# ryought/dbgphmm

Measured on AMD Instinct MI355X. Metric: read-bases/sec through forward+backward P(R|X), higher is better.
Workload: dtype f64

## Files before the change

dbgphmm_amd/_ffi.py:

```python
from __future__ import annotations

import ctypes as C
import os
import subprocess

_HERE = os.path.dirname(os.path.abspath(__file__))
LIB_PATH = os.environ.get("PHMM_AMD_LIB") or os.path.join(_HERE, "libphmm_amd.so")
CSRC = os.path.join(_HERE, "csrc")

PHMM_OK, PHMM_EINVAL, PHMM_ENODEVICE, PHMM_ENOMEM, PHMM_ECAPACITY, PHMM_EINTERNAL = 0, -1, -2, -3, -4, -5
PHMM_GROUP_MIXED = 0xFFFFFFFF
PHMM_STATS_DENSE_FWD, PHMM_STATS_DENSE_BWD, PHMM_STATS_SPARSE_FWD, PHMM_STATS_SPARSE_BWD, PHMM_STATS_HINTED_WIDE = range(5)
PHMM_READ_DEFERRED, PHMM_READ_WIDE_FRONTIER, PHMM_READ_FORCED_SWITCH = 1, 2, 4


class PhmmError(RuntimeError):
    def __init__(self, code: int, msg: str):
        super().__init__(f"phmm_amd error {code}: {msg}")
        self.code = code


def build(force: bool = False) -> str:
    if force:
        subprocess.check_call(["make", "-C", CSRC, "-s", "clean"])
# ... 59 lines not shown
        "phmm_full_prob_reads_copy_num_changes": (i32, [vp, vp, vp, vp, u32, u32, vp, vp, vp, vp, vp, vp]),
        "phmm_likelihood_create": (i32, [vp, vp, vp, vp, u32, P(vp)]),
        "phmm_likelihood_score_changes": (i32, [vp, u32, vp, vp, vp, vp, vp, vp]),
        "phmm_likelihood_move": (i32, [vp, u64, vp, vp, vp, vp]),
        "phmm_likelihood_current": (i32, [vp, vp, vp, vp]),
        "phmm_likelihood_refresh": (i32, [vp]),
        "phmm_likelihood_destroy": (None, [vp]),
        "phmm_likelihood_set_groups": (i32, [vp, u32, vp, vp]),
        "phmm_likelihood_score_group_changes": (i32, [vp, u32, vp, vp, vp, vp, vp, vp]),
        "phmm_likelihood_move_groups": (i32, [vp, u64, vp, vp, vp, vp]),
        "phmm_likelihood_current_groups": (i32, [vp, vp]),
        "phmm_generate_mappings": (i32, [vp, vp, vp, i32, P(vp), vp]),
        "phmm_run_with_mapping_edges": (i32, [vp, vp, vp, vp, vp, vp]),
        "phmm_last_call_stats": (i32, [i32, P(dbl), P(u64), P(u64)]),
        "phmm_enable_timing": (i32, [i32]),
    }
    for name, (res, args) in sig.items():
        fn = getattr(L, name)
        fn.restype = res
        fn.argtypes = args
    _lib = L
    return L


DECLARED_SYMBOLS = [
    "phmm_last_error", "phmm_version", "phmm_device_count", "phmm_set_device", "phmm_set_stream",
    "phmm_set_workspace_limit", "phmm_release_workspace", "phmm_workspace_bytes", "phmm_reads_last_call_info", "phmm_params_new", "phmm_params_uniform", "phmm_model_create",
    "phmm_model_set_probs", "phmm_model_set_params", "phmm_model_n_nodes", "phmm_model_n_edges",
    "phmm_model_destroy", "phmm_reads_create", "phmm_reads_count", "phmm_reads_total_bases",
    "phmm_reads_destroy", "phmm_run_dense", "phmm_run_dense_edges", "phmm_q_score_exact", "phmm_run_sparse", "phmm_full_prob_sparse_backward", "phmm_backward_sparse_tables", "phmm_dense_tables", "phmm_mappings_create",
# ... 6 lines not shown
    "phmm_likelihood_refresh", "phmm_likelihood_destroy",
    "phmm_likelihood_set_groups", "phmm_likelihood_score_group_changes", "phmm_likelihood_move_groups",
    "phmm_likelihood_current_groups",
]


def check(rc: int) -> None:
    if rc != PHMM_OK:
        raise PhmmError(rc, lib().phmm_last_error().decode())


def last_call_stats(which: int):
    ms, n, c = C.c_double(), C.c_uint64(), C.c_uint64()
    check(lib().phmm_last_call_stats(which, C.byref(ms), C.byref(n), C.byref(c)))
    return ms.value, n.value, c.value
```

dbgphmm_amd/csrc/api.cpp:

```cpp
#include <chrono>
#include <cstdlib>
#include <cmath>
#include <cstring>

#include "phmm_internal.h"

namespace phmm {

static thread_local std::string g_error;
static thread_local hipStream_t g_stream = nullptr;
static thread_local uint64_t g_ws_limit = 0;
static thread_local CallStats g_stats;
static thread_local bool g_timing = false;

void set_error(const std::string &msg) { g_error = msg; }
int fail(int code, const std::string &msg) {
    g_error = msg;
    return code;
}
hipStream_t current_stream() { return g_stream; }
int &workset_index() {
    static thread_local int idx = 0;
    return idx;
}
// ... 42 lines not shown
    k.no_wide_hinted = flag("PHMM_NO_WIDE_HINTED");
    k.wide_hinted = flag("PHMM_WIDE_HINTED") && !k.no_wide_hinted;
    k.no_wide_list_bwd = flag("PHMM_NO_WIDE_LIST_BWD");
    k.wide_hinted_cpb = num("PHMM_WIDE_HINTED_CPB", 0);
    if (k.wide_hinted_cpb != 1 && k.wide_hinted_cpb != 2 && k.wide_hinted_cpb != 4) k.wide_hinted_cpb = 0;
    k.no_side_worker = flag("PHMM_NO_SIDE_WORKER");
    k.no_wide_handover = flag("PHMM_NO_WIDE_HANDOVER");
    k.workers = std::max(1, std::min(MAX_WORKERS, num("PHMM_WORKERS", 1)));
    k.warm_cols = num("PHMM_WARM_COLS", 0);
    k.chunk_groups = std::max(0, num("PHMM_CHUNK_GROUPS", 0));
    k.no_keep_all = flag("PHMM_NO_KEEP_ALL");
    k.pipeline_min_groups = std::max(1, num("PHMM_PIPELINE_MIN_GROUPS", 8));
    k.no_runmax = flag("PHMM_NO_RUNMAX");
    k.force_radix = flag("PHMM_FORCE_RADIX");
    k.no_bwd_skip = flag("PHMM_NO_BWD_SKIP");
    k.serial_emit = flag("PHMM_SERIAL_EMIT");
    k.emit_high_priority = flag("PHMM_EMIT_HIGH_PRIORITY");
    k.no_dma = flag("PHMM_NO_DMA");
    k.bwd_dma = flag("PHMM_BWD_DMA");
    k.dense_streams = num("PHMM_DENSE_STREAMS", 0);
    k.dense_w = num("PHMM_DENSE_W", 0);
    k.dense_npt = num("PHMM_DENSE_NPT", 0);
    if (const char *e = std::getenv("PHMM_MEM_FRACTION")) k.mem_fraction = std::min(0.97, std::max(0.1, std::atof(e)));
    g_knobs = k;
}

void trace(const char *tag) {
    if (!g_knobs.trace) return;
    static thread_local std::chrono::steady_clock::time_point last = std::chrono::steady_clock::now();
    (void)hipStreamSynchronize(g_stream);
// ... 216 lines not shown
}
int phmm_set_workspace_limit(uint64_t bytes) {
    g_ws_limit = bytes;
    return PHMM_OK;
}
int phmm_enable_timing(int on) {
    g_timing = on != 0;
    return PHMM_OK;
}
int phmm_last_call_stats(int which, double *ms, uint64_t *launches, uint64_t *cells) {
    if (which < 0 || which > 4) return fail(PHMM_EINVAL, "which out of range");
    if (ms) *ms = g_stats.ms[which];
    if (launches) *launches = g_stats.launches[which];
    if (cells) *cells = g_stats.cells[which];
    return PHMM_OK;
}

static double lnz(double x) { return x > 0.0 ? std::log(x) : -INFINITY; }

int phmm_params_new(double p_mismatch, double p_gap_open, double p_gap_ext, double p_end,
                    int64_t n_active_nodes, int64_t n_warmup, phmm_params *o) {
    return guarded([&] {
        if (!o) PHMM_THROW(PHMM_EINVAL, "out is NULL");
        o->p_mismatch = lnz(p_mismatch);
        o->p_gap_open = lnz(p_gap_open);
        o->p_gap_ext = lnz(p_gap_ext);
        o->p_end = lnz(p_end);
        o->p_DD = o->p_II = o->p_gap_ext;
        o->p_MI = o->p_MD = o->p_ID = o->p_DI = o->p_gap_open;
        const double go = std::exp(o->p_gap_open), ge = std::exp(o->p_gap_ext), pe = std::exp(o->p_end);
// ... 650 lines not shown
```

dbgphmm_amd/csrc/dense.hip:

```cpp
#include <algorithm>
#include <cmath>
#include <cstring>
#include <numeric>
#include <type_traits>

#include "dense_internal.h"
#include "lds_dma.h"

#ifndef PHMM_FWD_PF
#define PHMM_FWD_PF 2
#endif
#ifndef PHMM_BWD_PF
#define PHMM_BWD_PF 1
#endif
#ifndef PHMM_SMALLW_WAVES
#define PHMM_SMALLW_WAVES 3
#endif

namespace phmm {


__device__ __forceinline__ int xcd_block(int b, int nblk8) {
    int per = nblk8 >> 3;
    return (b & 7) * per + (b >> 3);
// ... 749 lines not shown
    const double t2 = block_reduce_rows<W>(s2, OpAdd(), lds);
    if (threadIdx.x < W && lb < a.nblk) {
        double *bp = a.bpart + ((size_t)(pos & 1) * a.ng + g) * a.nblk8 * W * 2;
        bp[((size_t)lb * W + r) * 2 + 0] = t1;
        bp[((size_t)lb * W + r) * 2 + 1] = t2;
    }
    if (lb == 0 && threadIdx.x < W && live) a.BE[((size_t)g * (a.Lc + 1) + pos) * W + r] = Epos;
}

template <int W>
__global__ void __launch_bounds__(BLOCK) bwd_finish(const DenseArgs a) {
    __shared__ double lds[(BLOCK / 64) * 64];
    bwd_chain<W>(a, blockIdx.x, 0, lds);
}

__global__ void __launch_bounds__(BLOCK) freq_reduce(const double *accg, int ng, int N, double *out, int accumulate) {
    const int k = blockIdx.x * BLOCK + threadIdx.x;
    if (k >= N) return;
    double s = accumulate ? out[k] : 0.0;
    for (int g = 0; g < ng; g++) s += accg[(size_t)g * N + k];
    out[k] = s;
}

template <int W>
__global__ void __launch_bounds__(BLOCK) edge_freq_kernel(const DenseArgs a, const uint32_t *esrc, const uint32_t *edst,
                                                          const double *trans, const double *init, int E, double *accE,
                                                          double *accI) {
    constexpr int ROWS = BLOCK / W;
    const int g = blockIdx.y;
    const int r = threadIdx.x % W, row = threadIdx.x / W;
// ... 294 lines not shown
        if (w == 1 || w == 2 || w == 4 || w == 8 || w == 16 || w == 32 || w == 64) p.W = w;
    }
    p.ng_total = (int)((R + p.W - 1) / p.W);
    const int rows = BLOCK / p.W;
    int npt = 8;
    const double lanes_total = (double)m->N * (double)(p.ng_total * p.W);
    while (npt < 64 && lanes_total / (npt * 2) >= 524288.0) npt *= 2;
    while ((int64_t)((m->N + (int64_t)npt * rows - 1) / ((int64_t)npt * rows)) > 4096 && npt < 64) npt *= 2;
    if (knobs().dense_npt > 0) npt = std::max(2, std::min(256, knobs().dense_npt & ~1));
    p.npt = npt;
    p.nblk = (int)((m->N + (int64_t)npt * rows - 1) / ((int64_t)npt * rows));
    p.nblk8 = (p.nblk + 7) / 8 * 8;
    return p;
}

void layout(DenseArgs &a, int W, bool full_b, void *tables, void *misc, size_t &tb, size_t &mb, bool backward_only) {
    const size_t NW = (size_t)a.N * W;
    Carver t(tables), s(misc);
    const size_t fcols = backward_only ? 0 : (size_t)a.Lc;
    a.Fm = t.take<double>((size_t)a.ng * fcols * NW);
    a.Fi = t.take<double>((size_t)a.ng * fcols * NW);
    a.Fd = t.take<double>((size_t)a.ng * fcols * NW);
    a.bcols = full_b ? a.Lc : 2;
    a.Bm = t.take<double>((size_t)a.ng * a.bcols * NW);
    a.Bi = t.take<double>((size_t)a.ng * a.bcols * NW);
    a.Bd = (full_b || backward_only) ? t.take<double>((size_t)a.ng * a.bcols * NW) : nullptr;
    tb = t.off;
    a.bases = s.take<uint8_t>((size_t)a.ng * a.Lc * W);
    a.len = s.take<int>((size_t)a.ng * W);
    a.FE = s.take<int>((size_t)a.ng * (a.Lc + 1) * W);
    a.BE = s.take<int>((size_t)a.ng * (a.Lc + 1) * W);
    a.cmaxF = s.take<unsigned long long>((size_t)a.ng * a.Lc * W);
    a.cmaxB = s.take<unsigned long long>((size_t)a.ng * a.Lc * W);
    a.epart = s.take<double>((size_t)a.ng * (a.eall ? a.Lc : 1) * a.nblk8 * W);
    a.logPf = s.take<double>((size_t)a.ng * W);
    a.logE = s.take<double>(a.eall ? (size_t)a.ng * a.Lc * W : 1);
    a.bpart = s.take<double>((size_t)2 * a.ng * a.nblk8 * W * 2);
    a.logmbB = s.take<double>((size_t)a.ng * (a.Lc + 1) * W);
    a.logibB = s.take<double>((size_t)a.ng * (a.Lc + 1) * W);
    a.accg = s.take<double>((size_t)a.ng * a.N);
    a.logib = s.take<double>((size_t)a.Lc + 1);
    a.tmaxF = s.take<unsigned long long>((size_t)a.ng * a.Lc * W);
// ... 383 lines not shown
```

dbgphmm_amd/csrc/dense_internal.h:

```cpp
#pragma once

#include <vector>

#include "phmm_internal.h"
#include "seg_hull.h"

namespace phmm {

static constexpr double LN2 = 0.693147180559945309417232121458;
static constexpr int BLOCK = 256;

struct DenseArgs {
    int N, ng, Lc, nblk, npt;
    int g_off;
    const NodeRec *nodes;
    const uint8_t *emis;
    const double *init, *dinit, *tdinit;
    const uint32_t *fc_off;
    const FwdEntry *fc;
    const uint32_t *bc_off;
    const BwdEntry *bc;
    const uint32_t *fh_off, *bh_off;
    const HopEntry *fh, *bh;
    int hop_mode;
// ... 36 lines not shown
    uint8_t *skA = nullptr;
    int nrun = 0, nseg = 0, sseg = 1;
    unsigned long long *skcells = nullptr;
};
static constexpr int WF_CAP = 1024;


struct Plan {
    int W, ng_total, npt, nblk, nblk8;
    std::vector<uint32_t> order;
};

Plan make_plan(const phmm_model *m, const phmm_reads *reads, int forced_w);
Plan make_plan_ids(const phmm_model *m, const phmm_reads *reads, const std::vector<uint32_t> &ids);
void layout(DenseArgs &a, int W, bool full_b, void *tables, void *misc, size_t &tb, size_t &mb,
            bool backward_only = false);
void fill_model_args(DenseArgs &a, const phmm_model *m);
void host_logib(const phmm_model *m, size_t n, std::vector<double> &out);
void launch_fwd_step(int W, const DenseArgs &a, int pos);
void launch_fwd_finish(int W, const DenseArgs &a);
void launch_bwd_step(int W, const DenseArgs &a, int pos);
void launch_bwd_finish(int W, const DenseArgs &a);

struct ExactTables {
    double *f_m, *f_i, *f_d, *f_scal, *b_m, *b_i, *b_d, *b_scal;
};
void exact_dense_reads(phmm_model *m, const uint8_t *bases, const uint64_t *off, const std::vector<uint32_t> &ids, double *lf,
                       double *lb, double *freq_dev, const ExactTables *tabs, double *edge_freq_dev = nullptr,
                       double *init_freq_dev = nullptr);
bool certify_dense(int N, int len, double log2P, const int *FE, const double *log2maxF, const int *BE, const double *log2maxB,
                   double log2_p_end);
// ... 4 lines not shown
```

dbgphmm_amd/csrc/mapping_flow.hip:

```cpp
#include <algorithm>
#include <cmath>
#include <cstring>
#include <memory>

#include <hipcub/hipcub.hpp>

#include "sparse_dyn.h"
#include "lean_bwd_kernel.h"
#include "wide_bwd_kernel.h"

namespace phmm {

static constexpr int KMAX = PHMM_MAX_ACTIVE_NODES;

template <int CAP> struct FRec {
    double m[CAP], i[CAP], d[CAP];
    uint32_t id[CAP];
    int n, na, E;
};

template <int CAP> __device__ bool load_record(const RecPool &p, uint64_t pos_index, FRec<CAP> &f) {
    const uint64_t o1 = p.off[pos_index];
    if (o1 == 0) return false;
    const uint8_t *rec = p.base + (o1 - 8);
// ... 884 lines not shown
        pos_max = std::max(pos_max, hb[gi] & ~(1 << 30));
    }
    DevBuf &ctl = m->wset().aux[3], &pbuf = m->wset().aux[4];
    const bool skip = W == 64 && !knobs().no_bwd_skip && pos_max >= 0;
    const int sseg = seg_size(mc.a.npt);
    const RunSucc *rsucc = skip ? &model_run_successors(m, sseg) : nullptr;
    const size_t sk_nrun = ((size_t)m->N + mc.a.npt - 1) / mc.a.npt;
    size_t cb = 0;
    auto carve = [&](size_t bytes) {
        cb = (cb + 255) / 256 * 256;
        size_t o = cb;
        cb += bytes;
        return o;
    };
    const size_t o_bs = carve(sizeof(int) * lanes), o_ca = carve(sizeof(int) * lanes * 2), o_cb = carve(sizeof(int) * lanes * 2),
                 o_err = carve(sizeof(uint32_t) * lanes), o_cells = carve(sizeof(unsigned long long)), o_lanes = carve(sizeof(uint32_t) * std::max<size_t>(sparse_lanes.size(), 1)),
                 o_lp0 = carve(sizeof(uint64_t) * (lanes + 1)), o_gp0 = carve(sizeof(uint64_t) * (lanes + 1)),
                 o_stop = carve(sizeof(int) * lanes),
                 o_skh = carve(skip ? sizeof(uint32_t) * (size_t)mc.a.ng * rsucc->nseg : 0), o_ska = carve(skip ? 2 * (size_t)mc.a.ng * sk_nrun : 0),
                 o_bn = carve(sizeof(uint32_t) * (size_t)lanes * KMAX * 2), o_bv = carve(sizeof(double) * (size_t)lanes * KMAX * 2),
                 o_an = carve(sizeof(uint32_t) * (size_t)lanes * KMAX * 2), o_av = carve(sizeof(double) * (size_t)lanes * KMAX * 2),
                 o_hand = carve(sizeof(BHandoff) * (size_t)lanes), o_eoff = carve(sizeof(unsigned long long) * 2 * (size_t)lanes),
                 o_wls = carve(sizeof(uint32_t) * 2 * (size_t)lanes), o_wlb = carve(sizeof(uint32_t) * 2 * (size_t)lanes),
                 o_wlc = carve(sizeof(int) * 2), o_lb = carve(sizeof(double) * (size_t)lanes);
    ctl.reserve(cb);
    char *cp = (char *)ctl.p;
    const size_t prun_n = (size_t)mc.ngc * mc.a.nblk8 * BLOCK;
    bool need_pb = false;
    for (int gi = 0; gi < lanes; gi++) need_pb |= hb[gi] >= 0 && !(hb[gi] & (1 << 30));
    pbuf.reserve(((need_pb ? 3 : 2) * (size_t)mc.ngc * NW + prun_n) * sizeof(double));
    unsigned long long top_before = 0;
    HIP_CHECK(hipMemcpyAsync(&top_before, sink->mp.top, sizeof(top_before), hipMemcpyDeviceToHost, s));
    HIP_CHECK(hipStreamSynchronize(s));

    for (int attempt = 0;; attempt++) {
        HIP_CHECK(hipMemsetAsync(cp, 0, o_bn, s));
        HIP_CHECK(hipMemcpyAsync(cp + o_bs, hb.data(), sizeof(int) * lanes, hipMemcpyHostToDevice, s));
        HIP_CHECK(hipMemcpyAsync(cp + o_lp0, lp0.data(), sizeof(uint64_t) * (lanes + 1), hipMemcpyHostToDevice, s));
        HIP_CHECK(hipMemcpyAsync(cp + o_gp0, gp0.data(), sizeof(uint64_t) * (lanes + 1), hipMemcpyHostToDevice, s));
        if (!sparse_lanes.empty())
            HIP_CHECK(hipMemcpyAsync(cp + o_lanes, sparse_lanes.data(), sizeof(uint32_t) * sparse_lanes.size(),
                                     hipMemcpyHostToDevice, s));
        const RecPool mp = sink->mp;

        DenseArgs a = mc.a;
        a.want_freq = 0;
        a.want_map = 1;
        a.bstart = (const int *)(cp + o_bs);
        a.Pa = pbuf.as<double>();
        a.Pb = need_pb ? pbuf.as<double>() + 2 * (size_t)mc.ngc * NW : pbuf.as<double>();
        a.Prun = knobs().no_runmax ? nullptr : pbuf.as<double>() + (need_pb ? 3 : 2) * (size_t)mc.ngc * NW;
        const bool st_on = W == 64 && mc.main_plan;
        if (skip) {
            a.rs_off = rsucc->off.as<uint32_t>();
            a.rs = rsucc->ent.as<uint32_t>();
            a.nseg = (int)rsucc->nseg;
            a.sseg = sseg;
            a.nrun = (int)sk_nrun;
            a.skH = (uint32_t *)(cp + o_skh);
            a.skA = (uint8_t *)(cp + o_ska);
            a.skcells = st_on ? (unsigned long long *)(cp + o_cells) : nullptr;
            HIP_CHECK(hipMemsetAsync(pbuf.p, 0, sizeof(double) * 2 * (size_t)mc.ngc * NW, s));
        }
        HIP_CHECK(hipMemsetAsync(a.cmaxB, 0, sizeof(unsigned long long) * (size_t)a.ng * a.Lc * W, s));
        HIP_CHECK(hipMemsetAsync(a.pmax, 0, sizeof(unsigned long long) * (size_t)a.ng * (a.Lc + 1) * W, s));
        HIP_CHECK(hipMemsetAsync(a.BE, 0, sizeof(int) * (size_t)a.ng * (a.Lc + 1) * W, s));
        HIP_CHECK(hipMemsetAsync(a.Bm, 0, sizeof(double) * (size_t)a.ng * a.bcols * NW, s));
        HIP_CHECK(hipMemsetAsync(a.Bi, 0, sizeof(double) * (size_t)a.ng * a.bcols * NW, s));

        if (!sparse_lanes.empty()) {
            hipLaunchKernelGGL(merge_logp, dim3((unsigned)((sparse_lanes.size() + BLOCK - 1) / BLOCK)), dim3(BLOCK), 0, s,
                               (const uint32_t *)(cp + o_lanes), (int)sparse_lanes.size(), mc.d_logp_sparse, a.logPf);
            SparseBwdArgs ba{};
            ba.M = mc.fa_M;
            ba.d = a;
            ba.W = W;
            ba.Lb = mc.Lfull;
            ba.sw = mc.d_sw;
            ba.bases = mc.d_bases_full;
            ba.fpool = mc.fpool;
            ba.mpool = mp;
            ba.lane_pos0 = (const uint64_t *)(cp + o_lp0);
            ba.map_pos0 = (const uint64_t *)(cp + o_gp0);
// ... 91 lines not shown
        std::unique_lock<std::mutex> dense_lock;
        if (mc.dense_token) dense_lock = std::unique_lock<std::mutex>(*mc.dense_token);
        const int wi = workset_index();
        if (!m->pool->cstream[wi]) {
            int least = 0, greatest = 0;
            HIP_CHECK(hipDeviceGetStreamPriorityRange(&least, &greatest));
            HIP_CHECK(hipStreamCreateWithPriority(&m->pool->cstream[wi], hipStreamNonBlocking, knobs().emit_high_priority ? greatest : least));
        }
        for (auto &e : m->pool->cevent[wi])
            if (!e) HIP_CHECK(hipEventCreateWithFlags(&e, hipEventDisableTiming));
        hipStream_t s2 = knobs().serial_emit ? s : m->pool->cstream[wi];
        hipEvent_t *ev_col = &m->pool->cevent[wi][0], *ev_emit = &m->pool->cevent[wi][2];
        bool emitted[2] = {false, false};
        for (int pos = pos_max; pos >= 0; pos--) {
            const int par = pos & 1;
            a.Pa = pbuf.as<double>() + (size_t)par * mc.ngc * NW;
            ma.d = a;
            ma.cntA = (int *)(cp + o_ca) + (size_t)par * lanes;
            ma.cntB = (int *)(cp + o_cb) + (size_t)par * lanes;
            ma.candA_node = (uint32_t *)(cp + o_an) + (size_t)par * lanes * KMAX;
            ma.candA_val = (double *)(cp + o_av) + (size_t)par * lanes * KMAX;
            ma.candB_node = (uint32_t *)(cp + o_bn) + (size_t)par * lanes * KMAX;
            ma.candB_val = (double *)(cp + o_bv) + (size_t)par * lanes * KMAX;
            if (emitted[par]) HIP_CHECK(hipStreamWaitEvent(s, ev_emit[par], 0));
            lt.begin();
            launch_bwd_step(W, a, pos);
            lt.end();
            launch_post_collect_w(W, ma, pos);
            HIP_CHECK(hipEventRecord(ev_col[par], s));
            HIP_CHECK(hipStreamWaitEvent(s2, ev_col[par], 0));
            hipLaunchKernelGGL(emit_offsets, dim3(1), dim3(1024), 0, s2, ma, pos, lanes);
            {
                const int ub = std::max(1, live_at[(size_t)pos] * (need_pb ? 2 : 1));
                hipLaunchKernelGGL(emit_dense_small, dim3((unsigned)std::min(1024, (ub + BLOCK / 64 - 1) / (BLOCK / 64))), dim3(BLOCK), 0,
                                   s2, ma, pos, lanes);
                hipLaunchKernelGGL(emit_dense_map, dim3((unsigned)ub), dim3(BLOCK), 0, s2, ma, pos, lanes);
            }
            HIP_CHECK(hipEventRecord(ev_emit[par], s2));
            emitted[par] = true;
            if (st_on) st.launches[1]++;
        }
        for (int par = 0; par < 2; par++)
            if (emitted[par]) HIP_CHECK(hipStreamWaitEvent(s, ev_emit[par], 0));
        HIP_CHECK(hipGetLastError());
        const bool want_lb = mc.logb_out && pos_max >= 0 && lanes > 0;
        if (want_lb) {
            launch_bwd_finish(W, a);
            hipLaunchKernelGGL(gather_logb, dim3((unsigned)((lanes + BLOCK - 1) / BLOCK)), dim3(BLOCK), 0, s, (const double *)a.logmbB,
                               a.Lc, W, lanes, (double *)(cp + o_lb));
            HIP_CHECK(hipGetLastError());
        }
        st.ms[1] += lt.total_ms();
        for (int gi = 0; gi < lanes; gi++)
            if (st_on && !a.skcells && hb[gi] >= 0) st.cells[1] += (uint64_t)((hb[gi] & ~(1 << 30)) + 1) * m->N;
        const size_t err_words = (o_cells + sizeof(unsigned long long) - o_err) / sizeof(uint32_t);
        std::vector<uint32_t> herr(err_words);
        HIP_CHECK(hipMemcpyAsync(herr.data(), cp + o_err, sizeof(uint32_t) * err_words, hipMemcpyDeviceToHost, s));
        if (want_lb) HIP_CHECK(hipMemcpyAsync(mc.logb_out, cp + o_lb, sizeof(double) * lanes, hipMemcpyDeviceToHost, s));
        HIP_CHECK(hipStreamSynchronize(s));
        if (a.skcells) {
            unsigned long long nc = 0;
            memcpy(&nc, herr.data() + (o_cells - o_err) / sizeof(uint32_t), sizeof nc);
            st.cells[1] += nc;
        }
        if (dense_lock.owns_lock()) dense_lock.unlock();
        trace("  dense backward+collect");
        bool pool_full = false;
        for (int gi = 0; gi < lanes; gi++) {
            if (herr[gi] & SP_ERR_POOL) pool_full = true;
            else if (herr[gi] & ~SP_STOP_SLICE) PHMM_THROW(PHMM_EINTERNAL, "mapping backward error " + std::to_string(herr[gi]));
        }
        if (!pool_full) break;
        (void)attempt;
        throw SinkOverflow{};
    }
}

__global__ void __launch_bounds__(BLOCK) map_counts(RecPool mp, uint64_t n_pos, uint64_t *cnt) {
    const uint64_t p = (uint64_t)blockIdx.x * BLOCK + threadIdx.x;
    if (p > n_pos) return;
    uint64_t c = 0;
    if (p < n_pos) {
        const uint64_t o1 = mp.off[p];
        if (o1) c = ((const uint32_t *)(mp.base + (o1 - 8)))[0];
    }
    cnt[p] = c;
}
__global__ void __launch_bounds__(BLOCK) map_compact(RecPool mp, uint64_t n_pos, const uint64_t *pos_off, uint32_t *nodes,
                                                     double *logp) {
    const uint64_t p = (uint64_t)blockIdx.x * BLOCK + threadIdx.x;
// ... 692 lines not shown
```

dbgphmm_amd/csrc/phmm_internal.h:

```cpp
#pragma once

#include <hip/hip_runtime.h>

#include <cstdint>
#include <cstdio>
#include <memory>
#include <mutex>
#include <string>
#include <vector>

#include "../../include/phmm_amd.h"

namespace phmm {

void set_error(const std::string &msg);
int fail(int code, const std::string &msg);

struct Error {
    int code;
    std::string msg;
};
#define PHMM_THROW(code, msg) throw ::phmm::Error{(code), (msg)}
#define HIP_CHECK(expr)                                                                      \
    do {                                                                                     \
// ... 48 lines not shown
    }
    void *detach() {
        void *q = p;
        p = nullptr;
        bytes = 0;
        return q;
    }
    template <class T> T *as() const { return reinterpret_cast<T *>(p); }
    void upload(const void *src, size_t n) {
        reserve(n);
        if (n) HIP_CHECK(hipMemcpyAsync(p, src, n, hipMemcpyHostToDevice, current_stream()));
    }
};
void copy_out(void *dst, const void *src_dev, size_t bytes);

struct WorkSet {
    DevBuf tables, misc, aux[24];
    size_t bytes() const {
        size_t b = tables.bytes + misc.bytes;
        for (const auto &a : aux) b += a.bytes;
        return b;
    }
    void release() {
        tables.release();
        misc.release();
        for (auto &a : aux) a.release();
    }
};
static constexpr int MAX_WORKERS = 4;
struct DevicePool {
    int device = 0;
    std::recursive_mutex call_mu;
    WorkSet wsets[MAX_WORKERS];
    hipStream_t wstream[MAX_WORKERS] = {};
    hipStream_t cstream[MAX_WORKERS] = {};
    hipEvent_t cevent[MAX_WORKERS][4] = {};
    DevBuf ws_out;
    static constexpr size_t SPARE_MAX = 6, SPARE_BYTES = (size_t)8 << 30;
    std::mutex spare_mu;
    std::vector<std::pair<void *, size_t>> spare;
// ... 2 lines not shown
    void take(DevBuf &b, size_t n);
    void flush_spares();
    size_t owned_table_bytes() const {
        size_t b = 0;
        for (const auto &w : wsets) b += w.tables.bytes;
        return b;
    }
    size_t owned_bytes() const {
        size_t b = ws_out.bytes + spare_total;
        for (const auto &w : wsets) b += w.bytes();
        return b;
    }
    void release();
};
DevicePool &device_pool();

struct LinParams {
    double p_mismatch, p_match, p_random, p_end;
    double p_MM, p_IM, p_DM, p_MI, p_II, p_DI, p_MD, p_ID, p_DD;
    int n_max_gaps;
};

struct FwdEntry {
    uint32_t node;
    uint32_t pad;
    double w1, wD, wT;
};
struct BwdEntry {
    uint32_t node;
    uint32_t emis;
// ... 133 lines not shown
    std::vector<uint32_t> g_of;
    std::vector<uint32_t> g_cn;
    std::vector<uint32_t> g_emit;
    std::vector<uint32_t> g_seen;
    std::vector<uint32_t> g_at;
    uint32_t g_stamp = 0;
    phmm::DevBuf d_g_off, d_g_nodes, d_g_slot, d_bp_off, d_bp_slot;
};

namespace phmm {

struct CallStats {
    double ms[5] = {0, 0, 0, 0, 0};
    uint64_t launches[5] = {0, 0, 0, 0, 0};
    uint64_t cells[5] = {0, 0, 0, 0, 0};
};
CallStats &stats();
bool timing_enabled();

struct LaunchTimer {
    bool on;
    std::vector<hipEvent_t> ev;
    explicit LaunchTimer(bool on_) : on(on_) {}
    ~LaunchTimer() {
        for (auto e : ev) (void)hipEventDestroy(e);
    }
    void begin() {
        if (!on) return;
        hipEvent_t e;
        HIP_CHECK(hipEventCreate(&e));
// ... 30 lines not shown
    int wide_hinted_cpb = 0;
    bool no_side_worker = false;
    bool no_wide_handover = false;
    int workers = 1;
    int warm_cols = 0;
    int chunk_groups = 0;
    bool no_keep_all = false;
    int pipeline_min_groups = 8;
    bool no_runmax = false;
    bool force_radix = false;
    bool serial_emit = false;
    bool emit_high_priority = false;
    bool no_dma = false;
    bool bwd_dma = false;
    bool no_bwd_skip = false;
    int dense_streams = 0;
    int dense_w = 0;
    int dense_npt = 0;
    double mem_fraction = 0.0;
};
const Knobs &knobs();
void refresh_knobs();

void model_build_host(phmm_model *m);
void model_upload(phmm_model *m);
const RunSucc &model_run_successors(phmm_model *m, int seg);

void run_dense(phmm_model *m, const phmm_reads *reads, double *out_lf, double *out_lb,
               double *out_nf);
void full_prob_sparse_backward(phmm_model *m, const phmm_reads *reads, double *out_logp, double *out_total);
// ... 42 lines not shown
```

dbgphmm_amd/csrc/seg_hull.h:

```cpp
#pragma once

#if defined(__HIPCC__)
#define PHMM_SEG_FN __host__ __device__ inline
#else
#define PHMM_SEG_FN inline
#endif

namespace phmm {

static constexpr int SEGS_PER_RUN = 8;

PHMM_SEG_FN int seg_size(int npt) { return npt % SEGS_PER_RUN == 0 ? npt / SEGS_PER_RUN : npt; }

static constexpr int SEGS_PER_RUN_LOG2 = 3;
static_assert(SEGS_PER_RUN == 1 << SEGS_PER_RUN_LOG2, "a run's byte of A holds one bit per segment");
PHMM_SEG_FN int segs_per_run_log2(int npt) { return npt % SEGS_PER_RUN == 0 ? SEGS_PER_RUN_LOG2 : 0; }

PHMM_SEG_FN bool seg_hull(unsigned mask, int S, int jtop, int *first, int *top) {
    if (!mask) return false;
    const int lo = __builtin_ctz(mask), hi = 31 - __builtin_clz(mask);
    const int t = hi * S + S - 1;
    *first = lo * S;
    *top = (t < jtop ? t : jtop) - lo * S;
    return true;
}

}
```

dbgphmm_amd/csrc/sparse_dyn.hip:

```cpp
#include <algorithm>
#include <cmath>
#include <cstdlib>
#include <cstring>

#include "dense_internal.h"
#include <condition_variable>
#include <deque>
#include <exception>
#include <functional>
#include <memory>
#include <mutex>
#include <thread>

#include "frontier_dev.h"
#include "sparse_dyn.h"
#include "sparse_fwd_kernel.h"
#include "wide_fwd_kernel.h"
#include "lean_fwd_kernel.h"

namespace phmm {

struct WarmArgs {
    DenseArgs d;
    int *sw;
// ... 409 lines not shown
        const uint64_t R = plan.order.size();
        const int g0 = it.g0, ngc = it.ngc, Lc = it.Lc, Lfull = it.Lfull;
        std::vector<uint32_t> deferred_ids;
        std::vector<uint32_t> *deferred = it.pc->may_defer ? &deferred_ids : nullptr;
        DenseArgs base{};
        fill_model_args(base, m);
        base.nblk = plan.nblk;
        base.nblk8 = plan.nblk8;
        base.npt = plan.npt;
        base.eall = 0;
        base.want_freq = 0;
        {
        DenseArgs a = base;
        a.ng = ngc;
        a.Lc = Lc;
        size_t tb = 0, mb = 0;
        layout(a, W, false, nullptr, nullptr, tb, mb);
        m->wset().tables.reserve(tb);
        m->wset().misc.reserve(mb);
        layout(a, W, false, m->wset().tables.p, m->wset().misc.p, tb, mb);
        HIP_CHECK(hipMemsetAsync(m->wset().misc.p, 0, mb, s));
        const int lanes = ngc * W;
        size_t wb = 0;
        auto carve = [&](size_t bytes) {
            wb = (wb + 255) / 256 * 256;
            size_t o = wb;
            wb += bytes;
            return o;
        };
        const size_t o_sw = carve(sizeof(int) * lanes), o_cnt = carve(sizeof(int) * lanes),
                     o_cn = carve(sizeof(int) * lanes), o_und = carve(sizeof(int) * 2),
                     o_amb = carve(sizeof(int) * lanes), o_wsub = carve(sizeof(int) * lanes),
                     o_wcnt = carve(sizeof(int) * lanes), o_mode = carve((size_t)lanes),
                     o_cnode = carve(sizeof(uint32_t) * (size_t)lanes * PHMM_MAX_ACTIVE_NODES),
                     o_ctot = carve(sizeof(double) * (size_t)lanes * PHMM_MAX_ACTIVE_NODES),
// ... 443 lines not shown
        single_mode = true;
        worker_loop();
        {
            std::lock_guard<std::mutex> lk(mu);
            main_done = true;
        }
        cv.notify_all();
        if (side_started && side_thread.joinable()) {
            side_thread.join();
            CallStats &st = stats();
            for (int k = 0; k < 5; k++) {
                st.ms[k] += side_stats.ms[k];
                st.launches[k] += side_stats.launches[k];
                st.cells[k] += side_stats.cells[k];
            }
        }
    } else {
        HIP_CHECK(hipStreamSynchronize(current_stream()));
        const ThreadContext ctx = capture_thread_context();
        CallStats merged;
        for (int t = 0; t < n_threads; t++)
            if (!m->pool->wstream[t]) HIP_CHECK(hipStreamCreateWithFlags(&m->pool->wstream[t], hipStreamNonBlocking));
        std::vector<std::thread> threads;
        struct JoinAll {
            std::vector<std::thread> &t;
            ~JoinAll() {
                for (auto &th : t)
                    if (th.joinable()) th.join();
            }
        } join_all{threads};
        threads.reserve(n_threads);
        for (int t = 0; t < n_threads; t++) {
            threads.emplace_back([&, t]() {
                adopt_thread_context(ctx, m->pool->wstream[t], t);
                worker_loop();
                (void)hipStreamSynchronize(m->pool->wstream[t]);
                std::lock_guard<std::mutex> lk(mu);
                const CallStats &ws = stats();
                for (int k = 0; k < 5; k++) {
                    merged.ms[k] += ws.ms[k];
                    merged.launches[k] += ws.launches[k];
                    merged.cells[k] += ws.cells[k];
                }
            });
        }
        for (auto &th : threads) th.join();
        stats() = merged;
    }
    if (first_error) std::rethrow_exception(first_error);
    if (by_ratio) {
        reads->warm_hint = new_hint;
        reads->last_flags = new_flags;
    }
    double tot = 0.0;
    for (uint64_t r = 0; r < R; r++) tot += lf[r];
    put_doubles(out_logp, lf.data(), R);
    put_doubles(out_total, &tot, 1);
    if (out_logb) std::copy(lb.begin(), lb.end(), out_logb);
// ... 4 lines not shown
```

Baseline: 30.24 million.

## Keep backward B and Pa planes zero at rest instead of re-memsetting each call

Moves the mapping-backward B planes and Pa ping-pong planes into dedicated persistent buffers that track how many bytes are known to be clean. After each backward pass, a new kernel clears only the node ranges the skip hull actually touched, so the next call can skip the full-plane memsets. This cuts memset bandwidth per call. In exchange it adds an extra clear kernel, bookkeeping that must stay correct across retries and buffer growth, and debug stats plus a scan API.

```diff
diff --git a/dbgphmm_amd/_ffi.py b/dbgphmm_amd/_ffi.py
--- a/dbgphmm_amd/_ffi.py
+++ b/dbgphmm_amd/_ffi.py
@@ -97,6 +97,7 @@
         "phmm_run_with_mapping_edges": (i32, [vp, vp, vp, vp, vp, vp]),
         "phmm_last_call_stats": (i32, [i32, P(dbl), P(u64), P(u64)]),
         "phmm_enable_timing": (i32, [i32]),
+        "phmm_zero_at_rest_stats": (i32, [P(u64), P(u64), P(u64)]),
     }
     for name, (res, args) in sig.items():
         fn = getattr(L, name)
@@ -133,3 +134,9 @@
     ms, n, c = C.c_double(), C.c_uint64(), C.c_uint64()
     check(lib().phmm_last_call_stats(which, C.byref(ms), C.byref(n), C.byref(c)))
     return ms.value, n.value, c.value
+
+
+def zero_at_rest_stats(scan: bool = False):
+    ms, cl, nz = C.c_uint64(), C.c_uint64(), C.c_uint64()
+    check(lib().phmm_zero_at_rest_stats(C.byref(ms), C.byref(cl), C.byref(nz) if scan else None))
+    return (ms.value, cl.value, nz.value) if scan else (ms.value, cl.value)
diff --git a/dbgphmm_amd/csrc/api.cpp b/dbgphmm_amd/csrc/api.cpp
--- a/dbgphmm_amd/csrc/api.cpp
+++ b/dbgphmm_amd/csrc/api.cpp
@@ -4,6 +4,7 @@
 #include <cstring>
 
 #include "phmm_internal.h"
+#include "../../include/phmm_amd_debug.h"
 
 namespace phmm {
 
@@ -80,6 +81,7 @@
     k.no_runmax = flag("PHMM_NO_RUNMAX");
     k.force_radix = flag("PHMM_FORCE_RADIX");
     k.no_bwd_skip = flag("PHMM_NO_BWD_SKIP");
+    k.no_zero_at_rest = flag("PHMM_NO_ZERO_AT_REST");
     k.serial_emit = flag("PHMM_SERIAL_EMIT");
     k.emit_high_priority = flag("PHMM_EMIT_HIGH_PRIORITY");
     k.no_dma = flag("PHMM_NO_DMA");
@@ -326,6 +328,18 @@
     if (launches) *launches = g_stats.launches[which];
     if (cells) *cells = g_stats.cells[which];
     return PHMM_OK;
+}
+
+int phmm_zero_at_rest_stats(uint64_t *memset_bytes, uint64_t *cleared_bytes, uint64_t *nonzero_words) {
+    if (memset_bytes) *memset_bytes = g_stats.zr_memset;
+    if (cleared_bytes) *cleared_bytes = g_stats.zr_cleared;
+    if (!nonzero_words) return PHMM_OK;
+    return guarded([&] {
+        require_device();
+        DevicePool &pool = device_pool();
+        std::lock_guard<std::recursive_mutex> lk(pool.call_mu);
+        *nonzero_words = zero_at_rest_scan(pool);
+    });
 }
 
 static double lnz(double x) { return x > 0.0 ? std::log(x) : -INFINITY; }
diff --git a/dbgphmm_amd/csrc/dense.hip b/dbgphmm_amd/csrc/dense.hip
--- a/dbgphmm_amd/csrc/dense.hip
+++ b/dbgphmm_amd/csrc/dense.hip
@@ -787,6 +787,39 @@
     bwd_chain<W>(a, blockIdx.x, 0, lds);
 }
 
+struct ClearPlanes {
+    double *p[4];
+    int n;
+    size_t gstride;
+    unsigned long long *bytes;
+};
+__global__ void __launch_bounds__(BLOCK) clear_walked(const DenseArgs a, const ClearPlanes cp) {
+    const int g = blockIdx.y;
+    const int rho = blockIdx.x * (BLOCK / 64) + (threadIdx.x >> 6);
+    const int l = threadIdx.x & 63;
+    if (rho >= a.nrun) return;
+    const size_t par = (size_t)a.ng * a.nrun, gr = (size_t)g * a.nrun + rho;
+    int node0 = 0, rows = 0;
+    if (!run_clear_range(a.skA[gr], a.skA[par + gr], a.npt, a.N, rho, &node0, &rows)) return;
+    const size_t n2 = (size_t)rows * 32;
+    for (int k = 0; k < cp.n; k++) {
+        double2 *p = reinterpret_cast<double2 *>(cp.p[k] + (size_t)g * cp.gstride + (size_t)node0 * 64);
+        for (size_t i = l; i < n2; i += 64) p[i] = make_double2(0.0, 0.0);
+    }
+    if (l == 0 && cp.bytes) atomicAdd(cp.bytes, (unsigned long long)rows * 64 * sizeof(double) * cp.n);
+}
+void launch_clear_walked(const DenseArgs &a, double *const *planes, int n, size_t gstride, unsigned long long *bytes) {
+    ClearPlanes cp{};
+    if (n < 1 || n > 4 || !a.skA || a.nrun <= 0 || a.ng <= 0) PHMM_THROW(PHMM_EINTERNAL, "clear_walked: bad arguments");
+    for (int k = 0; k < n; k++) cp.p[k] = planes[k];
+    cp.n = n;
+    cp.gstride = gstride;
+    cp.bytes = bytes;
+    hipLaunchKernelGGL(clear_walked, dim3((unsigned)((a.nrun + BLOCK / 64 - 1) / (BLOCK / 64)), (unsigned)a.ng), dim3(BLOCK), 0,
+                       current_stream(), a, cp);
+    HIP_CHECK(hipGetLastError());
+}
+
 __global__ void __launch_bounds__(BLOCK) freq_reduce(const double *accg, int ng, int N, double *out, int accumulate) {
     const int k = blockIdx.x * BLOCK + threadIdx.x;
     if (k >= N) return;
@@ -1111,18 +1144,21 @@
     return p;
 }
 
-void layout(DenseArgs &a, int W, bool full_b, void *tables, void *misc, size_t &tb, size_t &mb, bool backward_only) {
+void layout(DenseArgs &a, int W, bool full_b, void *tables, void *misc, size_t &tb, size_t &mb, bool backward_only,
+            size_t *bb, void *bplanes) {
     const size_t NW = (size_t)a.N * W;
-    Carver t(tables), s(misc);
+    Carver t(tables), s(misc), b(bplanes);
+    Carver &tB = bb ? b : t;
     const size_t fcols = backward_only ? 0 : (size_t)a.Lc;
     a.Fm = t.take<double>((size_t)a.ng * fcols * NW);
     a.Fi = t.take<double>((size_t)a.ng * fcols * NW);
     a.Fd = t.take<double>((size_t)a.ng * fcols * NW);
     a.bcols = full_b ? a.Lc : 2;
-    a.Bm = t.take<double>((size_t)a.ng * a.bcols * NW);
-    a.Bi = t.take<double>((size_t)a.ng * a.bcols * NW);
+    a.Bm = tB.take<double>((size_t)a.ng * a.bcols * NW);
+    a.Bi = tB.take<double>((size_t)a.ng * a.bcols * NW);
     a.Bd = (full_b || backward_only) ? t.take<double>((size_t)a.ng * a.bcols * NW) : nullptr;
     tb = t.off;
+    if (bb) *bb = b.off;
     a.bases = s.take<uint8_t>((size_t)a.ng * a.Lc * W);
     a.len = s.take<int>((size_t)a.ng * W);
     a.FE = s.take<int>((size_t)a.ng * (a.Lc + 1) * W);
diff --git a/dbgphmm_amd/csrc/dense_internal.h b/dbgphmm_amd/csrc/dense_internal.h
--- a/dbgphmm_amd/csrc/dense_internal.h
+++ b/dbgphmm_amd/csrc/dense_internal.h
@@ -74,7 +74,8 @@
 Plan make_plan(const phmm_model *m, const phmm_reads *reads, int forced_w);
 Plan make_plan_ids(const phmm_model *m, const phmm_reads *reads, const std::vector<uint32_t> &ids);
 void layout(DenseArgs &a, int W, bool full_b, void *tables, void *misc, size_t &tb, size_t &mb,
-            bool backward_only = false);
+            bool backward_only = false, size_t *bb = nullptr, void *bplanes = nullptr);
+void launch_clear_walked(const DenseArgs &a, double *const *planes, int n, size_t gstride, unsigned long long *bytes);
 void fill_model_args(DenseArgs &a, const phmm_model *m);
 void host_logib(const phmm_model *m, size_t n, std::vector<double> &out);
 void launch_fwd_step(int W, const DenseArgs &a, int pos);
diff --git a/dbgphmm_amd/csrc/mapping_flow.hip b/dbgphmm_amd/csrc/mapping_flow.hip
--- a/dbgphmm_amd/csrc/mapping_flow.hip
+++ b/dbgphmm_amd/csrc/mapping_flow.hip
@@ -922,7 +922,7 @@
         return o;
     };
     const size_t o_bs = carve(sizeof(int) * lanes), o_ca = carve(sizeof(int) * lanes * 2), o_cb = carve(sizeof(int) * lanes * 2),
-                 o_err = carve(sizeof(uint32_t) * lanes), o_cells = carve(sizeof(unsigned long long)), o_lanes = carve(sizeof(uint32_t) * std::max<size_t>(sparse_lanes.size(), 1)),
+                 o_err = carve(sizeof(uint32_t) * lanes), o_cells = carve(sizeof(unsigned long long)), o_clr = carve(sizeof(unsigned long long)), o_lanes = carve(sizeof(uint32_t) * std::max<size_t>(sparse_lanes.size(), 1)),
                  o_lp0 = carve(sizeof(uint64_t) * (lanes + 1)), o_gp0 = carve(sizeof(uint64_t) * (lanes + 1)),
                  o_stop = carve(sizeof(int) * lanes),
                  o_skh = carve(skip ? sizeof(uint32_t) * (size_t)mc.a.ng * rsucc->nseg : 0), o_ska = carve(skip ? 2 * (size_t)mc.a.ng * sk_nrun : 0),
@@ -936,7 +936,26 @@
     const size_t prun_n = (size_t)mc.ngc * mc.a.nblk8 * BLOCK;
     bool need_pb = false;
     for (int gi = 0; gi < lanes; gi++) need_pb |= hb[gi] >= 0 && !(hb[gi] & (1 << 30));
-    pbuf.reserve(((need_pb ? 3 : 2) * (size_t)mc.ngc * NW + prun_n) * sizeof(double));
+    pbuf.reserve(((need_pb ? 1 : 0) * (size_t)mc.ngc * NW + prun_n) * sizeof(double));
+    ZeroBuf &zb = m->wset().bplanes, &zp = m->wset().paplanes;
+    const size_t pa_need = sizeof(double) * 2 * (size_t)mc.ngc * NW;
+    zp.reserve(pa_need);
+    if ((void *)mc.a.Bm != zb.buf.p || mc.a.bcols != 2) PHMM_THROW(PHMM_EINTERNAL, "mapping backward: B planes outside their buffer");
+    const size_t b_need = (size_t)((char *)(mc.a.Bi + (size_t)mc.a.ng * mc.a.bcols * NW) - (char *)zb.buf.p);
+    if (b_need > zb.buf.bytes) PHMM_THROW(PHMM_EINTERNAL, "mapping backward: B planes outgrow their buffer");
+    const bool zr = skip && !knobs().no_zero_at_rest;
+    double *const pa0 = zp.buf.as<double>();
+    const bool st_on = W == 64 && mc.main_plan;
+    auto begin_use = [&](ZeroBuf &z, size_t need, bool zero_it) {
+        const size_t known = knobs().no_zero_at_rest ? 0 : z.clean;
+        z.clean = 0;
+        if (zero_it && known < need) {
+            HIP_CHECK(hipMemsetAsync((char *)z.buf.p + known, 0, need - known, s));
+            if (st_on) st.zr_memset += need - known;
+        }
+        return zero_it ? std::max(known, need) : (size_t)0;
+    };
+    size_t b_zero = 0, pa_zero = 0;
     unsigned long long top_before = 0;
     HIP_CHECK(hipMemcpyAsync(&top_before, sink->mp.top, sizeof(top_before), hipMemcpyDeviceToHost, s));
     HIP_CHECK(hipStreamSynchronize(s));
@@ -955,10 +974,9 @@
         a.want_freq = 0;
         a.want_map = 1;
         a.bstart = (const int *)(cp + o_bs);
-        a.Pa = pbuf.as<double>();
-        a.Pb = need_pb ? pbuf.as<double>() + 2 * (size_t)mc.ngc * NW : pbuf.as<double>();
-        a.Prun = knobs().no_runmax ? nullptr : pbuf.as<double>() + (need_pb ? 3 : 2) * (size_t)mc.ngc * NW;
-        const bool st_on = W == 64 && mc.main_plan;
+        a.Pa = pa0;
+        a.Pb = need_pb ? pbuf.as<double>() : pa0;
+        a.Prun = knobs().no_runmax ? nullptr : pbuf.as<double>() + (need_pb ? 1 : 0) * (size_t)mc.ngc * NW;
         if (skip) {
             a.rs_off = rsucc->off.as<uint32_t>();
             a.rs = rsucc->ent.as<uint32_t>();
@@ -968,13 +986,12 @@
             a.skH = (uint32_t *)(cp + o_skh);
             a.skA = (uint8_t *)(cp + o_ska);
             a.skcells = st_on ? (unsigned long long *)(cp + o_cells) : nullptr;
-            HIP_CHECK(hipMemsetAsync(pbuf.p, 0, sizeof(double) * 2 * (size_t)mc.ngc * NW, s));
-        }
+        }
+        pa_zero = begin_use(zp, pa_need, skip);
         HIP_CHECK(hipMemsetAsync(a.cmaxB, 0, sizeof(unsigned long long) * (size_t)a.ng * a.Lc * W, s));
         HIP_CHECK(hipMemsetAsync(a.pmax, 0, sizeof(unsigned long long) * (size_t)a.ng * (a.Lc + 1) * W, s));
         HIP_CHECK(hipMemsetAsync(a.BE, 0, sizeof(int) * (size_t)a.ng * (a.Lc + 1) * W, s));
-        HIP_CHECK(hipMemsetAsync(a.Bm, 0, sizeof(double) * (size_t)a.ng * a.bcols * NW, s));
-        HIP_CHECK(hipMemsetAsync(a.Bi, 0, sizeof(double) * (size_t)a.ng * a.bcols * NW, s));
+        b_zero = begin_use(zb, b_need, true);
 
         if (!sparse_lanes.empty()) {
             hipLaunchKernelGGL(merge_logp, dim3((unsigned)((sparse_lanes.size() + BLOCK - 1) / BLOCK)), dim3(BLOCK), 0, s,
@@ -1096,7 +1113,7 @@
         bool emitted[2] = {false, false};
         for (int pos = pos_max; pos >= 0; pos--) {
             const int par = pos & 1;
-            a.Pa = pbuf.as<double>() + (size_t)par * mc.ngc * NW;
+            a.Pa = pa0 + (size_t)par * mc.ngc * NW;
             ma.d = a;
             ma.cntA = (int *)(cp + o_ca) + (size_t)par * lanes;
             ma.cntB = (int *)(cp + o_cb) + (size_t)par * lanes;
@@ -1122,8 +1139,17 @@
             emitted[par] = true;
             if (st_on) st.launches[1]++;
         }
+        unsigned long long *clr = st_on ? (unsigned long long *)(cp + o_clr) : nullptr;
+        if (zr) {
+            double *const bp[4] = {a.Bm, a.Bm + NW, a.Bi, a.Bi + NW};
+            launch_clear_walked(a, bp, 4, 2 * NW, clr);
+        }
         for (int par = 0; par < 2; par++)
             if (emitted[par]) HIP_CHECK(hipStreamWaitEvent(s, ev_emit[par], 0));
+        if (zr) {
+            double *const pp[2] = {pa0, pa0 + (size_t)mc.ngc * NW};
+            launch_clear_walked(a, pp, 2, NW, clr);
+        }
         HIP_CHECK(hipGetLastError());
         const bool want_lb = mc.logb_out && pos_max >= 0 && lanes > 0;
         if (want_lb) {
@@ -1135,7 +1161,7 @@
         st.ms[1] += lt.total_ms();
         for (int gi = 0; gi < lanes; gi++)
             if (st_on && !a.skcells && hb[gi] >= 0) st.cells[1] += (uint64_t)((hb[gi] & ~(1 << 30)) + 1) * m->N;
-        const size_t err_words = (o_cells + sizeof(unsigned long long) - o_err) / sizeof(uint32_t);
+        const size_t err_words = (o_clr + sizeof(unsigned long long) - o_err) / sizeof(uint32_t);
         std::vector<uint32_t> herr(err_words);
         HIP_CHECK(hipMemcpyAsync(herr.data(), cp + o_err, sizeof(uint32_t) * err_words, hipMemcpyDeviceToHost, s));
         if (want_lb) HIP_CHECK(hipMemcpyAsync(mc.logb_out, cp + o_lb, sizeof(double) * lanes, hipMemcpyDeviceToHost, s));
@@ -1145,6 +1171,12 @@
             memcpy(&nc, herr.data() + (o_cells - o_err) / sizeof(uint32_t), sizeof nc);
             st.cells[1] += nc;
         }
+        unsigned long long cleared = 0;
+        if (zr && clr) memcpy(&cleared, herr.data() + (o_clr - o_err) / sizeof(uint32_t), sizeof cleared);
+        st.zr_cleared += cleared;
+        if (knobs().trace && W == 64)
+            std::fprintf(stderr, "      zero at rest: %s, B + Pa planes %zu B, cleared %llu B (call so far: memset %llu B)\n",
+                         zr ? "on" : "off", b_need + pa_need, cleared, (unsigned long long)st.zr_memset);
         if (dense_lock.owns_lock()) dense_lock.unlock();
         trace("  dense backward+collect");
         bool pool_full = false;
@@ -1152,10 +1184,40 @@
             if (herr[gi] & SP_ERR_POOL) pool_full = true;
             else if (herr[gi] & ~SP_STOP_SLICE) PHMM_THROW(PHMM_EINTERNAL, "mapping backward error " + std::to_string(herr[gi]));
         }
-        if (!pool_full) break;
+        if (!pool_full) {
+            if (zr) {
+                zb.clean = b_zero;
+                zp.clean = pa_zero;
+            }
+            break;
+        }
         (void)attempt;
         throw SinkOverflow{};
     }
+}
+
+__global__ void __launch_bounds__(BLOCK) count_nonzero_words(const unsigned long long *p, size_t n, unsigned long long *out) {
+    unsigned long long c = 0;
+    for (size_t i = (size_t)blockIdx.x * BLOCK + threadIdx.x; i < n; i += (size_t)gridDim.x * BLOCK) c += p[i] != 0ull;
+    if (c) atomicAdd(out, c);
+}
+uint64_t zero_at_rest_scan(DevicePool &pool) {
+    HIP_CHECK(hipDeviceSynchronize());
+    DevBuf cnt;
+    cnt.reserve(sizeof(unsigned long long));
+    HIP_CHECK(hipMemset(cnt.p, 0, sizeof(unsigned long long)));
+    for (auto &w : pool.wsets)
+        for (ZeroBuf *z : {&w.bplanes, &w.paplanes}) {
+            const size_t n = std::min(z->clean, z->buf.bytes) / sizeof(unsigned long long);
+            if (!n) continue;
+            const unsigned nb = (unsigned)std::min<size_t>((n + BLOCK - 1) / BLOCK, 65536);
+            hipLaunchKernelGGL(count_nonzero_words, dim3(nb), dim3(BLOCK), 0, nullptr, z->buf.as<unsigned long long>(), n,
+                               cnt.as<unsigned long long>());
+            HIP_CHECK(hipGetLastError());
+        }
+    unsigned long long h = 0;
+    HIP_CHECK(hipMemcpy(&h, cnt.p, sizeof h, hipMemcpyDeviceToHost));
+    return h;
 }
 
 __global__ void __launch_bounds__(BLOCK) map_counts(RecPool mp, uint64_t n_pos, uint64_t *cnt) {
diff --git a/dbgphmm_amd/csrc/phmm_internal.h b/dbgphmm_amd/csrc/phmm_internal.h
--- a/dbgphmm_amd/csrc/phmm_internal.h
+++ b/dbgphmm_amd/csrc/phmm_internal.h
@@ -86,16 +86,32 @@
 };
 void copy_out(void *dst, const void *src_dev, size_t bytes);
 
+struct ZeroBuf {
+    DevBuf buf;
+    size_t clean = 0;
+    void reserve(size_t n) {
+        if (n <= buf.bytes) return;
+        clean = 0;
+        buf.reserve(n);
+    }
+    void release() {
+        clean = 0;
+        buf.release();
+    }
+};
 struct WorkSet {
     DevBuf tables, misc, aux[24];
+    ZeroBuf bplanes, paplanes;
     size_t bytes() const {
-        size_t b = tables.bytes + misc.bytes;
+        size_t b = tables.bytes + misc.bytes + bplanes.buf.bytes + paplanes.buf.bytes;
         for (const auto &a : aux) b += a.bytes;
         return b;
     }
     void release() {
         tables.release();
         misc.release();
+        bplanes.release();
+        paplanes.release();
         for (auto &a : aux) a.release();
     }
 };
@@ -128,6 +144,7 @@
     void release();
 };
 DevicePool &device_pool();
+uint64_t zero_at_rest_scan(DevicePool &pool);
 
 struct LinParams {
     double p_mismatch, p_match, p_random, p_end;
@@ -291,6 +308,7 @@
     double ms[5] = {0, 0, 0, 0, 0};
     uint64_t launches[5] = {0, 0, 0, 0, 0};
     uint64_t cells[5] = {0, 0, 0, 0, 0};
+    uint64_t zr_memset = 0, zr_cleared = 0;
 };
 CallStats &stats();
 bool timing_enabled();
@@ -351,6 +369,7 @@
     bool no_dma = false;
     bool bwd_dma = false;
     bool no_bwd_skip = false;
+    bool no_zero_at_rest = false;
     int dense_streams = 0;
     int dense_w = 0;
     int dense_npt = 0;
diff --git a/dbgphmm_amd/csrc/seg_hull.h b/dbgphmm_amd/csrc/seg_hull.h
--- a/dbgphmm_amd/csrc/seg_hull.h
+++ b/dbgphmm_amd/csrc/seg_hull.h
@@ -25,4 +25,14 @@
     return true;
 }
 
+PHMM_SEG_FN bool run_clear_range(unsigned m0, unsigned m1, int npt, int N, int rho, int *node0, int *rows) {
+    const int kb = rho * npt;
+    const int jtop = npt - 1 < N - 1 - kb ? npt - 1 : N - 1 - kb;
+    int first = 0, top = -1;
+    if (jtop < 0 || !seg_hull(m0 | m1, seg_size(npt), jtop, &first, &top) || top < 0) return false;
+    *node0 = kb + first;
+    *rows = top + 1;
+    return true;
 }
+
+}
diff --git a/dbgphmm_amd/csrc/sparse_dyn.hip b/dbgphmm_amd/csrc/sparse_dyn.hip
--- a/dbgphmm_amd/csrc/sparse_dyn.hip
+++ b/dbgphmm_amd/csrc/sparse_dyn.hip
@@ -447,11 +447,13 @@
         DenseArgs a = base;
         a.ng = ngc;
         a.Lc = Lc;
-        size_t tb = 0, mb = 0;
-        layout(a, W, false, nullptr, nullptr, tb, mb);
+        size_t tb = 0, mb = 0, bb = 0;
+        ZeroBuf &bplanes = m->wset().bplanes;
+        layout(a, W, false, nullptr, nullptr, tb, mb, false, sink ? &bb : nullptr, nullptr);
         m->wset().tables.reserve(tb);
         m->wset().misc.reserve(mb);
-        layout(a, W, false, m->wset().tables.p, m->wset().misc.p, tb, mb);
+        if (sink) bplanes.reserve(bb);
+        layout(a, W, false, m->wset().tables.p, m->wset().misc.p, tb, mb, false, sink ? &bb : nullptr, bplanes.buf.p);
         HIP_CHECK(hipMemsetAsync(m->wset().misc.p, 0, mb, s));
         const int lanes = ngc * W;
         size_t wb = 0;
@@ -925,6 +927,8 @@
                 st.launches[k] += side_stats.launches[k];
                 st.cells[k] += side_stats.cells[k];
             }
+            st.zr_memset += side_stats.zr_memset;
+            st.zr_cleared += side_stats.zr_cleared;
         }
     } else {
         HIP_CHECK(hipStreamSynchronize(current_stream()));
@@ -953,6 +957,8 @@
                     merged.launches[k] += ws.launches[k];
                     merged.cells[k] += ws.cells[k];
                 }
+                merged.zr_memset += ws.zr_memset;
+                merged.zr_cleared += ws.zr_cleared;
             });
         }
         for (auto &th : threads) th.join();
diff --git a/include/phmm_amd_debug.h b/include/phmm_amd_debug.h
--- /dev/null
+++ b/include/phmm_amd_debug.h
@@ -0,0 +1,13 @@
+#ifndef PHMM_AMD_DEBUG_H
+#define PHMM_AMD_DEBUG_H
+#include <stdint.h>
+#ifdef __cplusplus
+extern "C" {
+#endif
+
+int phmm_zero_at_rest_stats(uint64_t *out_memset_bytes, uint64_t *out_cleared_bytes, uint64_t *out_nonzero_words);
+
+#ifdef __cplusplus
+}
+#endif
+#endif
```

Result: no change. 30.22 million (-0.0%).
